# chao1224/GeoSSL

Measured on AMD Instinct MI355X. Metric: molecules/s/GPU SchNet+DDM fwd+bwd (QM9-sized, bs=1024); % HBM roofline, higher is better.
Workload: dtype f32

## Files before the change

### geossl_amd/csrc/ncsn_bwd.hip

```cpp
#include "common.h"
#include "geossl_hip.h"
#include "split.h"
#include "tn.h"

using namespace geossl;

namespace {

constexpr int TR = 32;

#ifdef NB_TIMING
__device__ long long nb_dbg[2 * 32 * 8];
#define NB_MARK(slot)                                                                              \
  do {                                                                                             \
    if (blockIdx.x == 5 && lane == 0 && (wave == 0 || wave == NW) && t - t_begin < 32)             \
      nb_dbg[((wave == 0 ? 0 : 1) * 32 + (t - t_begin)) * 8 + (slot)] = clock64();                 \
  } while (0)
#else
#define NB_MARK(slot) do {} while (0)
#endif

template <int NW>
struct NbLds {
  static constexpr int F = 32 * NW, H = F / 2, KHS = (H + 15) / 16, HMB = (H + 31) / 32, KS = F / 16;
  u32x4* zb;
  u32x4* dz2T;
  u32x4* fT;
  u32x4* dz1r;
  u32x4* abT;
  int4* scal;
  float* pdv;
  float* dep;
  float* wls;
  int* eg;
  int* ef;
  int* ea;
  int* ec;
  __device__ explicit NbLds(uint8_t* smem) {
    zb = reinterpret_cast<u32x4*>(smem);
    dz2T = zb + 2 * KHS * 2 * 64;
    fT = dz2T + HMB * 2 * 2 * 64;
    dz1r = fT + 2 * NW * 2 * 2 * 64;
    abT = dz1r + KS * 2 * 64;
    scal = reinterpret_cast<int4*>(abT + NW * 2 * 2 * 64);
    pdv = reinterpret_cast<float*>(scal + 3 * TR);
    dep = pdv + 3 * TR;
    wls = dep + NW * TR;
    eg = reinterpret_cast<int*>(wls + F);
    ef = eg + 4;
    ea = ef + 2 * NW;
    ec = ea + NW;
  }
  static size_t bytes() {
    return (size_t)(2 * KHS * 2 + HMB * 4 + 2 * NW * 4 + KS * 2 + NW * 4) * 1024 + 3 * TR * sizeof(int4) +
           (size_t)(3 * TR + NW * TR + F) * sizeof(float) + (size_t)(4 + 4 * NW) * sizeof(int);
  }
};

struct NcsnFusedArgs {
  const float* h;
  const int64_t* sei0;
  const int64_t* sei1;
  int S;
  GeosslNcsnWeights w;
  GeosslNcsnSaved sv;
  const int64_t* divisor;
  float out_scale;
  const float* gout;
  float* dfeat;
  float* demb;
  float* grow;
  float* pw1;
  float* pd1;
  float* pb1;
  float* pw2;
  float* pb2;
  float* psm;
};

__device__ __forceinline__ float ldg_off(const float* base, uint32_t byte_off) {
  return *reinterpret_cast<const float*>(reinterpret_cast<const char*>(base) + byte_off);
}
__device__ __forceinline__ int crow4(int r, int k4) { return (r & 3) + 8 * (r >> 2) + k4; }
__device__ __forceinline__ int opaque(int v) {
  asm volatile("" : "+v"(v));
  return v;
}
__device__ __forceinline__ u32x4 pack8(const f32x16& t, int s) {
  u32x4 w;
#pragma unroll
  for (int q = 0; q < 4; ++q) {
    const f16x2 p = {(_Float16)t[8 * s + 2 * q], (_Float16)t[8 * s + 2 * q + 1]};
    w[q] = __builtin_bit_cast(uint32_t, p);
  }
  return w;
}
__device__ __forceinline__ const u32x4& piece(const Frag2& f, int pc) { return pc == 0 ? f.h : f.l; }
__device__ __forceinline__ int scale_exponent(float m) { return max(mag_exponent(m), -40); }
__device__ __forceinline__ float pow2(int e) { return __builtin_amdgcn_ldexpf(1.0f, e); }
constexpr int E_NONE = -100000;

template <int NW, bool ROLE_A>
__device__ __forceinline__ void ncsn_bwd_body(const NcsnFusedArgs& a, const int S, const float* __restrict__ a_h) {
  using L_t = NbLds<NW>;
  constexpr int F = L_t::F, H = L_t::H, KHS = L_t::KHS, HMB = L_t::HMB, KS = L_t::KS, NT = 128 * NW;
  extern __shared__ __attribute__((aligned(16))) uint8_t smem_raw[];
  const L_t L(smem_raw);
  const int tid = threadIdx.x, lane = tid & 63, j = lane & 31, kh = lane >> 5;
  const int wave = __builtin_amdgcn_readfirstlane(tid >> 6);
  const int nb = ROLE_A ? wave : wave - NW;
  const int ntiles = (S + TR - 1) / TR;
  const int per = (ntiles + (int)gridDim.x - 1) / (int)gridDim.x;
  const int t_begin = (int)blockIdx.x * per, t_end = min(ntiles, t_begin + per);
  const float scale = a.out_scale * (a.gout != nullptr ? a.gout[0] : 1.0f) / (float)a.divisor[0];
  const uint32_t col = 32 * nb + j;

  Frag2 wreg[ROLE_A ? KHS : KS];
  f32x16 accw1[ROLE_A ? NW : 1];
  f32x16 accw2[ROLE_A ? 1 : HMB];
  int E1[ROLE_A ? NW : 1];
  int E2 = E_NONE;
  int ew = 0;
  float bsum = 0.0f, dsum = 0.0f;
  u32x4 ident[2];
  float w3r[8];
  float s_w2 = 0.0f, s_w1 = 0.0f, s_b1 = 0.0f, s_g = 0.0f, s_d = 0.0f;
  float iw1 = 0.0f, ib1 = 0.0f, iw2 = 0.0f;
  int e3;
  {
    float m3 = 0.0f;
    for (int i = lane; i < H; i += 64) m3 = fmaxf(m3, fabsf(a.w.o3_w[i]));
    e3 = scale_exponent(wave_max(m3));
  }
  if constexpr (ROLE_A) {
    iw1 = a.w.in_w1[col];
    ib1 = a.w.in_b1[col];
    iw2 = a.w.in_w2[col];
    float raw[KHS][8];
    float wm = 0.0f, csum = 0.0f;
#pragma unroll
    for (int ks = 0; ks < KHS; ++ks)
#pragma unroll
      for (int e = 0; e < 8; ++e) {
        const int m = 16 * ks + 8 * kh + e;
        const float v = m < H ? a.w.o2_w[(size_t)m * F + col] : 0.0f;
        raw[ks][e] = v;
        wm = fmaxf(wm, fabsf(v));
        csum = fmaf(fabsf(v), m < H ? fabsf(a.w.o3_w[m]) : 0.0f, csum);
      }
    ew = scale_exponent(wave_max(wm));
    const float sw = pow2(14 - ew);
#pragma unroll
    for (int ks = 0; ks < KHS; ++ks) wreg[ks] = split8h_scaled(raw[ks], sw);
    csum += __shfl_xor(csum, 32, 64);
    const int ecw = max(mag_exponent(wave_max(csum)), -80);
    if (lane == 0) L.ec[nb] = ecw;
#pragma unroll
    for (int kb = 0; kb < NW; ++kb) {
      E1[kb] = E_NONE;
#pragma unroll
      for (int r = 0; r < 16; ++r) accw1[kb][r] = 0.0f;
    }
#pragma unroll
    for (int s = 0; s < 2; ++s)
#pragma unroll
      for (int q = 0; q < 4; ++q) {
        const int k0 = 16 * s + kperm(2 * q, kh), k1 = 16 * s + kperm(2 * q + 1, kh);
        ident[s][q] = (k0 == j ? 0x3C00u : 0u) | (k1 == j ? 0x3C000000u : 0u);
      }
// ... 18 lines not shown
    }
#pragma unroll
    for (int mb = 0; mb < HMB; ++mb)
#pragma unroll
      for (int r = 0; r < 16; ++r) accw2[mb][r] = 0.0f;
#pragma unroll
    for (int q2 = 0; q2 < 2; ++q2)
#pragma unroll
      for (int q = 0; q < 4; ++q) {
        const int k0 = 16 * q2 + 8 * kh + 2 * q;
        ident[q2][q] = (k0 == j ? 0x3C00u : 0u) | (k0 + 1 == j ? 0x3C000000u : 0u);
      }
  }
  for (int i = tid; i < F; i += NT) L.wls[i] = a.w.o1_w[(size_t)i * (F + 1) + F];

  int sc_u = 0, sc_v = 0;
  float sc_g = 0.0f, sc_e = 0.0f, sc_p = 0.0f;
  int EG = -60;
  auto load_scal = [&](int tt) {
    if constexpr (ROLE_A) {
      if (wave == 0) {
        const int row = min(TR * tt + j, S - 1);
        sc_u = (int)a.sei0[row];
        sc_v = (int)a.sei1[row];
        sc_g = a.sv.gscale[row];
        sc_e = a.sv.emb[row];
        sc_p = a.sv.pd[row];
      }
    }
  };
  auto put_scal = [&](int tt) {
    if constexpr (ROLE_A) {
      if (wave == 0) {
        const int row = TR * tt + lane;
        const bool valid = lane < TR && row < S && tt < t_end;
        const float gr = valid ? pin(sc_g) * scale : 0.0f;
        EG = max(EG, mag_exponent(wave_max(fabsf(gr))));
        if (lane < TR) {
          L.scal[(tt % 3) * TR + lane] = make_int4(sc_u, sc_v, __float_as_int(gr), __float_as_int(sc_e));
          L.pdv[(tt % 3) * TR + lane] = sc_p;
          if (valid) a.grow[row] = gr;
        }
        if (lane == 0) L.eg[tt % 3] = EG;
      }
    }
  };
  float a1raw[16];
  auto request_a1 = [&](int tt, int k4) {
    if constexpr (ROLE_A) {
#pragma unroll
      for (int r = 0; r < 16; ++r)
        a1raw[r] = ldg_off(a.sv.a1, ((uint32_t)min(TR * tt + crow4(r, k4), S - 1) * (uint32_t)F + col) * 4u);
    }
  };
  f32x4 a2raw[2];
  float o3acc[8] = {0.0f, 0.0f, 0.0f, 0.0f, 0.0f, 0.0f, 0.0f, 0.0f};
  auto request_a2 = [&](int tt) {
    if constexpr (!ROLE_A) {
      if (nb < KHS) {
        const uint32_t off = ((uint32_t)min(TR * tt + j, S - 1) * (uint32_t)H + (16 * nb + 8 * kh)) * 4u;
        a2raw[0] = *reinterpret_cast<const f32x4*>(reinterpret_cast<const char*>(a.sv.a2) + off);
        a2raw[1] = *reinterpret_cast<const f32x4*>(reinterpret_cast<const char*>(a.sv.a2) + 16 + off);
      }
    }
  };
  float hu[16], hv[16];
  auto request_gather = [&](int tt, int k4) {
    if constexpr (!ROLE_A) {
      const int2* sc = reinterpret_cast<const int2*>(L.scal + (tt % 3) * TR);
#pragma unroll
      for (int r = 0; r < 16; ++r) {
        const int2 uv = sc[2 * crow4(r, k4)];
        hu[r] = ldg_off(a_h, ((uint32_t)uv.x * (uint32_t)F + col) * 4u);
        hv[r] = ldg_off(a_h, ((uint32_t)uv.y * (uint32_t)F + col) * 4u);
      }
    }
  };
  auto build_zb = [&](int tt) {
    if constexpr (!ROLE_A) {
      if (nb < KHS) {
        const float gr = __int_as_float(L.scal[(tt % 3) * TR + j].z);
        const float sz = pow2(14 - e3 - __builtin_amdgcn_readfirstlane(L.eg[tt % 3]));
        const float av[8] = {a2raw[0].x, a2raw[0].y, a2raw[0].z, a2raw[0].w, a2raw[1].x, a2raw[1].y, a2raw[1].z, a2raw[1].w};
        float v[8];
#pragma unroll
        for (int e = 0; e < 8; ++e) {
          const float a2v = pin(av[e]);
          v[e] = a2v > 0.0f ? gr * w3r[e] : 0.0f;
          o3acc[e] = fmaf(gr, a2v, o3acc[e]);
        }
        const Frag2 f = split8h_scaled(v, sz);
        u32x4* dst = L.zb + (size_t)(((tt & 1) * KHS + nb) * 2) * 64 + lane;
        dst[0] = f.h;
        dst[64] = f.l;
      }
    }
  };
  int EF = -40;
  auto build_fT = [&](int tt) {
    if constexpr (!ROLE_A) {
      float v[16];
      float m = 0.0f;
#pragma unroll
      for (int r = 0; r < 16; ++r) {
        v[r] = pin(hu[r]) + pin(hv[r]);
        m = fmaxf(m, fabsf(v[r]));
      }
      EF = max(EF, mag_exponent(wave_max(m)));
      const float sf = pow2(14 - EF);
      if (lane == 0) L.ef[(tt & 1) * NW + nb] = EF;
#pragma unroll
      for (int s = 0; s < 2; ++s) {
        float vv[8];
#pragma unroll
        for (int e = 0; e < 8; ++e) vv[e] = v[8 * s + e];
        const Frag2 f = split8h_scaled(vv, sf);
        u32x4* dst = L.fT + (size_t)((((tt & 1) * NW + nb) * 2 + s) * 2) * 64 + lane;
        dst[0] = f.h;
        dst[64] = f.l;
      }
    }
  };

  load_scal(t_begin);
  put_scal(t_begin);
  load_scal(t_begin + 1);
  put_scal(t_begin + 1);
  load_scal(t_begin + 2);
  if (t_begin < t_end) {
    request_a1(t_begin, 4 * kh);
    request_a2(t_begin);
  }
  __syncthreads();
  int eC = -80;
#pragma unroll
  for (int i = 0; i < NW; ++i) eC = max(eC, __builtin_amdgcn_readfirstlane(L.ec[i]));
  if (t_begin < t_end) {
    request_gather(t_begin, 4 * kh);
    build_zb(t_begin);
    build_fT(t_begin);
    request_a2(t_begin + 1);
    request_gather(t_begin + 1, 4 * kh);
  }
  int EA = -40;
  const float kA = pow2(e3 + ew - eC - 14);
  for (int t = t_begin; t < t_end; ++t) {
    const int buf = t & 1;
    int k4 = opaque(4 * kh);
    NB_MARK(0);
    lds_barrier();
    NB_MARK(1);
    const int EGt = __builtin_amdgcn_readfirstlane(L.eg[t % 3]);
    if constexpr (ROLE_A) {
      put_scal(t + 2);
      const float kT = pow2(EGt + eC - 14);
      f32x16 acc0, acc1;
#pragma unroll
      for (int r = 0; r < 16; ++r) acc0[r] = acc1[r] = 0.0f;
      {
        const u32x4* zs = L.zb + (size_t)(buf * KHS * 2) * 64 + lane;
        Frag2 a0, an;
        a0.h = zs[0]; a0.l = zs[64];
#pragma unroll
        for (int ks = 0; ks < KHS; ++ks) {
          if (ks + 1 < KHS) {
            const u32x4* s0 = zs + (size_t)((ks + 1) * 2) * 64;
            an.h = s0[0]; an.l = s0[64];
          }
          __builtin_amdgcn_sched_barrier(0);
          mma3x2(acc0, acc1, a0, wreg[ks]);
          __builtin_amdgcn_sched_barrier(0);
          if (ks + 1 < KHS) a0 = an;
        }
      }
      NB_MARK(5);
      float v[16];
      {
        const int4* sc = L.scal + (t % 3) * TR;
        float tb = 0.0f, td = 0.0f, am = 0.0f;
#pragma unroll
        for (int r = 0; r < 16; ++r) {
          a1raw[r] = pin(a1raw[r]);
          v[r] = a1raw[r] > 0.0f ? (acc0[r] + acc1[r]) * kA : 0.0f;
          tb += v[r];
          td = fmaf(v[r], __int_as_float(sc[crow4(r, k4)].w), td);
          am = fmaxf(am, fabsf(a1raw[r]));
        }
        bsum = fmaf(tb, kT, bsum);
        dsum = fmaf(td, kT, dsum);
        EA = max(EA, mag_exponent(wave_max(am)));
      }
      {
        const float sa = pow2(14 - EA);
        if (lane == 0) L.ea[nb] = EA;
#pragma unroll
        for (int s = 0; s < 2; ++s) {
          float vv[8];
#pragma unroll
          for (int e = 0; e < 8; ++e) vv[e] = a1raw[8 * s + e];
          const Frag2 f = split8h_scaled(vv, sa);
          u32x4* dst = L.abT + (size_t)((nb * 2 + s) * 2) * 64 + lane;
          dst[0] = f.h;
          dst[64] = f.l;
        }
      }
      Frag2 da[2];
#pragma unroll
      for (int s = 0; s < 2; ++s) {
        float vv[8];
#pragma unroll
        for (int e = 0; e < 8; ++e) vv[e] = v[8 * s + e];
        da[s] = split8h(vv);
      }
      {
        float wl[16];
#pragma unroll
        for (int r = 0; r < 16; ++r) wl[r] = L.wls[32 * nb + crow4(r, k4)];
        float de = 0.0f;
#pragma unroll
        for (int pc = 1; pc >= 0; --pc) {
          f32x16 tp;
#pragma unroll
          for (int r = 0; r < 16; ++r) tp[r] = 0.0f;
          tp = mfma_f16(piece(da[0], pc), ident[0], tp);
          tp = mfma_f16(piece(da[1], pc), ident[1], tp);
#pragma unroll
          for (int r = 0; r < 16; ++r) de = fmaf(tp[r], wl[r], de);
#pragma unroll
          for (int half = 0; half < 2; ++half)
            L.dz1r[(size_t)((2 * nb + half) * 2 + pc) * 64 + lane] = pack8(tp, half);
        }
        de += __shfl_xor(de, 32, 64);
        if (kh == 0) L.dep[j * NW + nb] = de * kT;
      }
      NB_MARK(6);
#pragma unroll
      for (int kb = 0; kb < NW; ++kb) {
        const int En = EGt + __builtin_amdgcn_readfirstlane(L.ef[buf * NW + kb]);
        if (En != E1[kb]) {
          const float f = pow2(max(E1[kb] - En, -200));
#pragma unroll
          for (int r = 0; r < 16; ++r) accw1[kb][r] *= f;
          E1[kb] = En;
        }
#pragma unroll
        for (int s = 0; s < 2; ++s) {
          const u32x4* s0 = L.fT + (size_t)(((buf * NW + kb) * 2 + s) * 2) * 64 + lane;
          Frag2 bf;
          bf.h = s0[0]; bf.l = s0[64];
          mma3(accw1[kb], da[s], bf);
        }
      }
    } else {
      if (nb < HMB) {
        float tb = 0.0f;
#pragma unroll
        for (int pc = 1; pc >= 0; --pc) {
          f32x16 tp;
#pragma unroll
          for (int r = 0; r < 16; ++r) tp[r] = 0.0f;
#pragma unroll
          for (int q = 0; q < 2; ++q) {
            if (2 * nb + q < KHS) {
              const u32x4* s0 = L.zb + (size_t)((buf * KHS + 2 * nb + q) * 2 + pc) * 64 + lane;
              tp = mfma_f16(s0[0], ident[q], tp);
            }
          }
#pragma unroll
          for (int r = 0; r < 16; ++r) tb += tp[r];
#pragma unroll
          for (int s = 0; s < 2; ++s) L.dz2T[(size_t)((nb * 2 + s) * 2 + pc) * 64 + lane] = pack8(tp, s);
        }
        bsum = fmaf(tb, pow2(EGt + e3 - 14), bsum);
      }
      NB_MARK(5);
      build_zb(t + 1);
      NB_MARK(6);
      build_fT(t + 1);
    }
    k4 = opaque(4 * kh);
    NB_MARK(2);
    lds_barrier();
    NB_MARK(3);
    if constexpr (ROLE_A) {
      request_a1(t + 1, k4);
      load_scal(t + 3);
      {
        const int4* sc = L.scal + (t % 3) * TR;
        const float* pdr = L.pdv + (t % 3) * TR;
#pragma unroll
        for (int i = 0; i < 16; ++i) {
          const int rl = 4 * k4 + i;
          float de = 0.0f;
#pragma unroll
          for (int n2 = 0; n2 < NW; ++n2) de += L.dep[rl * NW + n2];
          const float pd = pdr[rl];
          const float pre = fmaf(iw1, pd, ib1);
          s_w2 = fmaf(de, fmaxf(pre, 0.0f), s_w2);
          const float dp = pre > 0.0f ? de * iw2 : 0.0f;
          s_w1 = fmaf(dp, pd, s_w1);
          s_b1 += dp;
          if (wave == 0 && j == i) {
            s_g += __int_as_float(sc[rl].z);
            s_d += de;
          }
        }
      }
    } else {
      request_a2(t + 2);
      request_gather(t + 2, k4);
      NB_MARK(7);
      f32x16 acc0, acc1;
#pragma unroll
      for (int r = 0; r < 16; ++r) acc0[r] = acc1[r] = 0.0f;
      {
        const u32x4* zs = L.dz1r + lane;
        Frag2 b0, bn;
        b0.h = zs[0]; b0.l = zs[64];
#pragma unroll
        for (int ks = 0; ks < KS; ++ks) {
          if (ks + 1 < KS) {
            const u32x4* s0 = zs + (size_t)((ks + 1) * 2) * 64;
            bn.h = s0[0]; bn.l = s0[64];
          }
          __builtin_amdgcn_sched_barrier(0);
          mma3x2(acc0, acc1, wreg[ks], b0);
          __builtin_amdgcn_sched_barrier(0);
          if (ks + 1 < KS) b0 = bn;
        }
      }
      const float kD = pow2(EGt + eC + ew - 28);
      f32x16 outp;
#pragma unroll
      for (int r = 0; r < 16; ++r) outp[r] = (acc0[r] + acc1[r]) * kD;
      const int row = TR * t + j;
      if (row < S) {
        const uint32_t off = ((uint32_t)row * (uint32_t)F + 32 * nb + 4 * kh) * 4u;
#pragma unroll
        for (int q = 0; q < 4; ++q)
          *reinterpret_cast<f32x4*>(reinterpret_cast<char*>(a.dfeat) + 32 * q + off) =
              f32x4{outp[4 * q], outp[4 * q + 1], outp[4 * q + 2], outp[4 * q + 3]};
        if (nb == 0 && kh == 0) {
          float de = 0.0f;
#pragma unroll
          for (int n2 = 0; n2 < NW; ++n2) de += L.dep[j * NW + n2];
          a.demb[row] = de;
        }
      }
      {
        const int En = EGt + __builtin_amdgcn_readfirstlane(L.ea[nb]);
        if (En != E2) {
          const float f = pow2(max(E2 - En, -200));
#pragma unroll
          for (int mb = 0; mb < HMB; ++mb)
#pragma unroll
            for (int r = 0; r < 16; ++r) accw2[mb][r] *= f;
          E2 = En;
        }
      }
#pragma unroll
      for (int s = 0; s < 2; ++s) {
        const u32x4* sb = L.abT + (size_t)((nb * 2 + s) * 2) * 64 + lane;
        Frag2 bf;
        bf.h = sb[0]; bf.l = sb[64];
#pragma unroll
        for (int mb = 0; mb < HMB; ++mb) {
          const u32x4* s0 = L.dz2T + (size_t)((mb * 2 + s) * 2) * 64 + lane;
          Frag2 af;
          af.h = s0[0]; af.l = s0[64];
          mma3(accw2[mb], af, bf);
        }
      }
    }
    NB_MARK(4);
  }
  const size_t pb = blockIdx.x;
  if constexpr (ROLE_A) {
    float* P1 = a.pw1 + pb * F * F;
#pragma unroll
    for (int kb = 0; kb < NW; ++kb) {
      const float f = pow2(max(E1[kb] + eC - 28, -200));
#pragma unroll
      for (int r = 0; r < 16; ++r) P1[(size_t)(32 * nb + c_row(r, lane)) * F + 32 * kb + j] = accw1[kb][r] * f;
    }
    const float sb = bsum + __shfl_xor(bsum, 32, 64), sd = dsum + __shfl_xor(dsum, 32, 64);
    if (kh == 0) {
      a.pb1[pb * F + col] = sb;
      a.pd1[pb * F + col] = sd;
    }
    float* Ps = a.psm + pb * (H + 3 * F + 2);
    const float t_w2 = s_w2 + __shfl_xor(s_w2, 32, 64);
    const float t_w1 = s_w1 + __shfl_xor(s_w1, 32, 64), t_b1 = s_b1 + __shfl_xor(s_b1, 32, 64);
    if (kh == 0) {
      Ps[H + col] = t_w2;
      Ps[H + F + col] = t_w1;
      Ps[H + 2 * F + col] = t_b1;
    }
    if (wave == 0) {
      const float tg = wave_sum(s_g), td = wave_sum(s_d);
      if (lane == 0) {
        Ps[H + 3 * F] = tg;
        Ps[H + 3 * F + 1] = td;
      }
    }
  } else {
    float* P2 = a.pw2 + pb * H * F;
    const float f = pow2(max(E2 + e3 - 28, -200));
#pragma unroll
    for (int mb = 0; mb < HMB; ++mb)
#pragma unroll
      for (int r = 0; r < 16; ++r) {
        const int m = 32 * mb + c_row(r, lane);
        if (m < H) P2[(size_t)m * F + col] = accw2[mb][r] * f;
      }
    const float sb = bsum + __shfl_xor(bsum, 32, 64);
    if (nb < HMB && kh == 0 && (int)col < H) a.pb2[pb * H + col] = sb;
    if (nb < KHS) {
      float* Ps = a.psm + pb * (H + 3 * F + 2);
#pragma unroll
      for (int e = 0; e < 8; ++e) {
        float v = o3acc[e];
#pragma unroll
        for (int o = 16; o > 0; o >>= 1) v += __shfl_xor(v, o, 64);
        const int m = 16 * nb + 8 * kh + e;
        if (j == 0 && m < H) Ps[m] = v;
      }
    }
  }
}

template <int NW>
__global__ __launch_bounds__(128 * NW) void k_ncsn_bwd_fused(NcsnFusedArgs a) {
  if ((int)(threadIdx.x >> 6) < NW) ncsn_bwd_body<NW, true>(a, a.S, a.h);
  else ncsn_bwd_body<NW, false>(a, a.S, a.h);
}
struct NcsnFusedPair { NcsnFusedArgs a[2]; };
template <int NW>
__global__ __launch_bounds__(128 * NW) void k_ncsn_bwd_fused2(NcsnFusedPair pr, const int32_t* __restrict__ dyn_S,
                                                              const int32_t* __restrict__ dyn_view) {
  const NcsnFusedArgs& a = pr.a[blockIdx.y];
  const int S = dyn_count(a.S, dyn_S);
  const float* h = a.h;
  if (dyn_view != nullptr && blockIdx.y == 1) h += (size_t)(*dyn_view) * (32 * NW);
  if ((int)(threadIdx.x >> 6) < NW) ncsn_bwd_body<NW, true>(a, S, h);
  else ncsn_bwd_body<NW, false>(a, S, h);
}

__device__ __forceinline__ void ncsn_reduce_all_block(const ReduceMulti& m, int nblk, int accumulate,
                                                      const float* __restrict__ psm, int F, const GeosslNcsnGrads& g,
                                                      float (*red)[64]) {
  const int mb = m.xoff[m.nseg];
  if ((int)blockIdx.x < mb) {
    reduce_multi_block(m, nblk, accumulate, red, 0);
    return;
  }
  const int H = F / 2, len = H + 3 * F + 2;
  const int i = ((int)blockIdx.x - mb) * 4 + (int)(threadIdx.x >> 6), lane = threadIdx.x & 63;
  if (i >= len) return;
  float s = 0.0f;
  for (int b = lane; b < nblk; b += 64) s += psm[(size_t)b * len + i];
  s = wave_sum(s);
  if (lane == 0) {
    float* dst;
    if (i < H) dst = g.o3_w + i;
    else if (i < H + F) dst = g.in_w2 + (i - H);
    else if (i < H + 2 * F) dst = g.in_w1 + (i - H - F);
    else if (i < H + 3 * F) dst = g.in_b1 + (i - H - 2 * F);
    else if (i == H + 3 * F) dst = g.o3_b;
    else dst = g.in_b2;
    *dst = accumulate ? *dst + s : s;
  }
}
__global__ __launch_bounds__(256) void k_ncsn_reduce_all(ReduceMulti m, int nblk, int accumulate,
                                                         const float* __restrict__ psm, int F, GeosslNcsnGrads g) {
  __shared__ float red[4][64];
  ncsn_reduce_all_block(m, nblk, accumulate, psm, F, g, red);
}
__global__ __launch_bounds__(256) void k_ncsn_reduce_all2(ReduceMulti m0, ReduceMulti m1, int nblk, int accumulate,
                                                          const float* __restrict__ psm0,
                                                          const float* __restrict__ psm1, int F, GeosslNcsnGrads g0,
                                                          GeosslNcsnGrads g1) {
  __shared__ float red[4][64];
  if (blockIdx.y == 0) ncsn_reduce_all_block(m0, nblk, accumulate, psm0, F, g0, red);
  else ncsn_reduce_all_block(m1, nblk, accumulate, psm1, F, g1, red);
}

inline int fused_blocks(int64_t S) {
  const int64_t ntiles = (S + TR - 1) / TR;
  return (int)(ntiles < 256 ? ntiles : 256);
}

}

#ifdef NB_TIMING
extern "C" int geossl_ncsn_bwd_debug_read(long long* host) {
  return (int)hipMemcpyFromSymbol(host, HIP_SYMBOL(nb_dbg), sizeof(long long) * 2 * 32 * 8);
}
#endif

extern "C" int64_t geossl_ddm_loss_bwd_fused_workspace_floats(int64_t S, int F) {
  const int64_t nb = fused_blocks(S), H = F / 2;
  return nb * ((int64_t)F * F + 2 * F + H * F + H + (H + 3 * F + 2));
}

extern "C" int geossl_ddm_loss_bwd_fused(const float* h, const int64_t* sei0, const int64_t* sei1, int64_t S, int64_t N,
                                         int F, const GeosslNcsnWeights* w, const GeosslNcsnSaved* saved,
                                         const int64_t* stats_divisor, float out_scale, const float* gout, float* dfeat,
                                         float* demb, float* grow, const GeosslNcsnGrads* grads, float* workspace,
                                         int accumulate, hipStream_t stream) {
  if (S <= 0) return 0;
  if (F != 32 && F != 64 && F != 128) return (int)hipErrorInvalidValue;
  if (S * (int64_t)F * 4 >= ((int64_t)1 << 32) || N * (int64_t)F * 4 >= ((int64_t)1 << 32)) return (int)hipErrorInvalidValue;
  const int nb = fused_blocks(S), H = F / 2;
  NcsnFusedArgs a;
  a.h = h; a.sei0 = sei0; a.sei1 = sei1; a.S = (int)S; a.w = *w; a.sv = *saved; a.divisor = stats_divisor;
  a.out_scale = out_scale; a.gout = gout; a.dfeat = dfeat; a.demb = demb; a.grow = grow;
  a.pw1 = workspace;
  a.pd1 = a.pw1 + (size_t)nb * F * F;
  a.pb1 = a.pd1 + (size_t)nb * F;
  a.pw2 = a.pb1 + (size_t)nb * F;
  a.pb2 = a.pw2 + (size_t)nb * H * F;
  a.psm = a.pb2 + (size_t)nb * H;
#define LAUNCH(NWV)                                                                                      \
  do {                                                                                                   \
    allow_big_lds(&k_ncsn_bwd_fused<NWV>);                                                               \
// ... 91 lines not shown
```

### geossl_amd/csrc/ncsn_rows.hip

```cpp
#include "common.h"
#include "geossl_hip.h"
#include "split.h"

using namespace geossl;

namespace {

struct RowIn {
  int64_t u, v;
  float sigma, d, eps;
};

template <int NMB>
__device__ __forceinline__ void ncsn_fwd_body(const float* __restrict__ h, const int64_t* __restrict__ batch,
                                              const int64_t* __restrict__ sei0, const int64_t* __restrict__ sei1,
                                              int S, const float* __restrict__ distance,
                                              const int64_t* __restrict__ noise_level,
                                              const float* __restrict__ dist_noise, const GeosslNcsnWeights& w,
                                              float anneal_power, float* __restrict__ loss_e,
                                              const GeosslNcsnSaved& sv, float* __restrict__ loss_part) {
  constexpr int F = 32 * NMB, H = F / 2, HMB = (H + 31) / 32, HP = 32 * HMB, KS = F / 16;
  extern __shared__ __attribute__((aligned(16))) uint8_t smem_raw[];
  u32x4* W1f = reinterpret_cast<u32x4*>(smem_raw);
  u32x4* W2f = W1f + NMB * KS * 3 * 64;
  float* b1s = reinterpret_cast<float*>(W2f + HMB * KS * 3 * 64);
  float* wls = b1s + F;
  float* b2s = wls + F;
  float* w3s = b2s + HP;
  float* iw1 = w3s + HP;
  float* ib1 = iw1 + F;
  float* iw2 = ib1 + F;
  float* lred = iw2 + F;
  const int tid = threadIdx.x, lane = tid & 63, wave = tid >> 6, j = lane & 31, kh = lane >> 5;
  const int nrb = (S + 31) / 32;
  float lsum = 0.0f;
  auto load_row = [&](int rb) {
    RowIn r;
    const int rowc = min(32 * rb + j, S - 1);
    r.u = sei0[rowc];
    r.v = sei1[rowc];
    r.sigma = w.sigmas[noise_level[batch[r.u]]];
    r.d = distance[rowc];
    r.eps = dist_noise[rowc];
    return r;
  };
  int rb = blockIdx.x + gridDim.x * wave;
  RowIn cur;
  if (rb < nrb) cur = load_row(rb);
#ifdef NCSN_STAGE_UNROLL
#pragma unroll
#endif
  for (int i = tid; i < NMB * KS * 64; i += 512) {
    const int ln = i & 63, ks = (i >> 6) % KS, mb = i / (64 * KS);
    const float* row = w.o1_w + (size_t)(32 * mb + (ln & 31)) * (F + 1) + 16 * ks + 8 * (ln >> 5);
    float v[8];
#pragma unroll
    for (int e = 0; e < 8; ++e) v[e] = row[e];
    const Frag3 f = split8(v);
    u32x4* dst = W1f + ((size_t)(mb * KS + ks) * 3) * 64 + ln;
    dst[0] = f.h;
    dst[64] = f.m;
    dst[128] = f.l;
  }
#ifdef NCSN_STAGE_UNROLL
#pragma unroll
#endif
  for (int i = tid; i < HMB * KS * 64; i += 512) {
    const int ln = i & 63, ks = (i >> 6) % KS, mb = i / (64 * KS);
    const int m = 32 * mb + (ln & 31);
    const float* row = w.o2_w + (size_t)min(m, H - 1) * F + 16 * ks + 4 * (ln >> 5);
    const f32x4 lo = *reinterpret_cast<const f32x4*>(row), hi = *reinterpret_cast<const f32x4*>(row + 8);
    float v[8] = {lo.x, lo.y, lo.z, lo.w, hi.x, hi.y, hi.z, hi.w};
    if (m >= H) {
#pragma unroll
      for (int e = 0; e < 8; ++e) v[e] = 0.0f;
    }
    const Frag3 f = split8(v);
    u32x4* dst = W2f + ((size_t)(mb * KS + ks) * 3) * 64 + ln;
    dst[0] = f.h;
    dst[64] = f.m;
    dst[128] = f.l;
  }
  for (int i = tid; i < F; i += 512) {
    b1s[i] = w.o1_b[i];
    wls[i] = w.o1_w[(size_t)i * (F + 1) + F];
    iw1[i] = w.in_w1[i];
    ib1[i] = w.in_b1[i];
    iw2[i] = w.in_w2[i];
  }
  for (int i = tid; i < HP; i += 512) {
    b2s[i] = i < H ? w.o2_b[i] : 0.0f;
    w3s[i] = i < H ? w.o3_w[i] : 0.0f;
  }
  __syncthreads();
  const float ib2 = w.in_b2[0], b3 = w.o3_b[0];
  for (; rb < nrb; rb += gridDim.x * 8) {
    const int row = 32 * rb + j;
    const bool valid = row < S;
    const RowIn in = cur;
    f32x4 gq[2][4];
    auto gather = [&](int ks, f32x4 (&g)[4]) {
      const float* hu = h + (size_t)in.u * F + 16 * ks + 8 * kh;
      const float* hv = h + (size_t)in.v * F + 16 * ks + 8 * kh;
      g[0] = *reinterpret_cast<const f32x4*>(hu);
      g[1] = *reinterpret_cast<const f32x4*>(hu + 4);
      g[2] = *reinterpret_cast<const f32x4*>(hv);
      g[3] = *reinterpret_cast<const f32x4*>(hv + 4);
    };
    gather(0, gq[0]);
    if (rb + gridDim.x * 8 < nrb) cur = load_row(rb + gridDim.x * 8);
    const float pd = add_rn(in.d, mul_rn(in.eps, in.sigma));
    float e = 0.0f;
#pragma unroll 4
    for (int k = kh * (F / 2); k < (kh + 1) * (F / 2); k += 4) {
      const f32x4 a = *reinterpret_cast<const f32x4*>(iw1 + k), b = *reinterpret_cast<const f32x4*>(ib1 + k);
      const f32x4 c = *reinterpret_cast<const f32x4*>(iw2 + k);
      e = fmaf(c.x, fmaxf(fmaf(a.x, pd, b.x), 0.0f), e);
      e = fmaf(c.y, fmaxf(fmaf(a.y, pd, b.y), 0.0f), e);
      e = fmaf(c.z, fmaxf(fmaf(a.z, pd, b.z), 0.0f), e);
      e = fmaf(c.w, fmaxf(fmaf(a.w, pd, b.w), 0.0f), e);
    }
    e += __shfl_xor(e, 32, 64);
    const float emb = e + ib2;
    f32x16 acc1[NMB];
#pragma unroll
    for (int mb = 0; mb < NMB; ++mb)
#pragma unroll
      for (int q = 0; q < 4; ++q) {
        const f32x4 b = *reinterpret_cast<const f32x4*>(b1s + 32 * mb + 8 * q + 4 * kh);
        const f32x4 wl = *reinterpret_cast<const f32x4*>(wls + 32 * mb + 8 * q + 4 * kh);
        acc1[mb][4 * q] = fmaf(emb, wl.x, b.x);
        acc1[mb][4 * q + 1] = fmaf(emb, wl.y, b.y);
        acc1[mb][4 * q + 2] = fmaf(emb, wl.z, b.z);
        acc1[mb][4 * q + 3] = fmaf(emb, wl.w, b.w);
      }
#pragma unroll
    for (int ks = 0; ks < KS; ++ks) {
      if (ks + 1 < KS) gather(ks + 1, gq[(ks + 1) & 1]);
      const f32x4(&g)[4] = gq[ks & 1];
      const float v[8] = {g[0].x + g[2].x, g[0].y + g[2].y, g[0].z + g[2].z, g[0].w + g[2].w,
                          g[1].x + g[3].x, g[1].y + g[3].y, g[1].z + g[3].z, g[1].w + g[3].w};
      const Frag3 bf = split8(v);
      Frag3 af[NMB];
#pragma unroll
      for (int mb = 0; mb < NMB; ++mb) {
        const u32x4* src = W1f + ((size_t)(mb * KS + ks) * 3) * 64 + lane;
        af[mb].h = src[0];
        af[mb].m = src[64];
        af[mb].l = src[128];
      }
#pragma unroll
      for (int mb = 0; mb < NMB; ++mb) acc1[mb] = mfma_bf16(af[mb].l, bf.h, acc1[mb]);
#pragma unroll
      for (int mb = 0; mb < NMB; ++mb) acc1[mb] = mfma_bf16(af[mb].h, bf.l, acc1[mb]);
#pragma unroll
      for (int mb = 0; mb < NMB; ++mb) acc1[mb] = mfma_bf16(af[mb].m, bf.m, acc1[mb]);
#pragma unroll
      for (int mb = 0; mb < NMB; ++mb) acc1[mb] = mfma_bf16(af[mb].m, bf.h, acc1[mb]);
#pragma unroll
      for (int mb = 0; mb < NMB; ++mb) acc1[mb] = mfma_bf16(af[mb].h, bf.m, acc1[mb]);
#pragma unroll
      for (int mb = 0; mb < NMB; ++mb) acc1[mb] = mfma_bf16(af[mb].h, bf.h, acc1[mb]);
      __builtin_amdgcn_sched_barrier(0);
    }
    Frag3 tb[KS];
    {
      float* arow = sv.a1 != nullptr ? sv.a1 + (size_t)row * F + 4 * kh : nullptr;
#pragma unroll
      for (int mb = 0; mb < NMB; ++mb)
#pragma unroll
        for (int half = 0; half < 2; ++half) {
          float v[8];
#pragma unroll
          for (int e2 = 0; e2 < 8; ++e2) v[e2] = fmaxf(acc1[mb][8 * half + e2], 0.0f);
          if (arow != nullptr && valid) {
            *reinterpret_cast<f32x4*>(arow + 32 * mb + 16 * half) = f32x4{v[0], v[1], v[2], v[3]};
            *reinterpret_cast<f32x4*>(arow + 32 * mb + 16 * half + 8) = f32x4{v[4], v[5], v[6], v[7]};
          }
          tb[2 * mb + half] = split8(v);
          __builtin_amdgcn_sched_barrier(0);
        }
    }
    float sc = 0.0f;
#pragma unroll
    for (int mb = 0; mb < HMB; ++mb) {
      f32x16 acc2;
#pragma unroll
      for (int q = 0; q < 4; ++q) {
        const f32x4 b = *reinterpret_cast<const f32x4*>(b2s + 32 * mb + 8 * q + 4 * kh);
        acc2[4 * q] = b.x;
        acc2[4 * q + 1] = b.y;
        acc2[4 * q + 2] = b.z;
        acc2[4 * q + 3] = b.w;
      }
      Frag3 af, an;
      {
        const u32x4* src = W2f + ((size_t)(mb * KS) * 3) * 64 + lane;
        af.h = src[0]; af.m = src[64]; af.l = src[128];
      }
#pragma unroll
      for (int ks = 0; ks < KS; ++ks) {
        if (ks + 1 < KS) {
          const u32x4* src = W2f + ((size_t)(mb * KS + ks + 1) * 3) * 64 + lane;
          an.h = src[0]; an.m = src[64]; an.l = src[128];
        }
        __builtin_amdgcn_sched_barrier(0);
        mma6(acc2, af, tb[ks]);
        __builtin_amdgcn_sched_barrier(0);
        if (ks + 1 < KS) af = an;
      }
      float* a2row = sv.a2 != nullptr ? sv.a2 + (size_t)row * H + 32 * mb + 4 * kh : nullptr;
#pragma unroll
      for (int q = 0; q < 4; ++q) {
        const f32x4 w3 = *reinterpret_cast<const f32x4*>(w3s + 32 * mb + 8 * q + 4 * kh);
        const f32x4 a = f32x4{fmaxf(acc2[4 * q], 0.0f), fmaxf(acc2[4 * q + 1], 0.0f), fmaxf(acc2[4 * q + 2], 0.0f),
                              fmaxf(acc2[4 * q + 3], 0.0f)};
        sc = fmaf(a.x, w3.x, sc);
        sc = fmaf(a.y, w3.y, sc);
        sc = fmaf(a.z, w3.z, sc);
        sc = fmaf(a.w, w3.w, sc);
        if (a2row != nullptr && valid && 32 * mb + 8 * q + 4 * kh < H) *reinterpret_cast<f32x4*>(a2row + 8 * q) = a;
      }
    }
    sc += __shfl_xor(sc, 32, 64);
    const float out = sc + b3;
    const float inv_sigma = 1.0f / in.sigma;
    const float score = out * inv_sigma;
    const float target = (-1.0f / (in.sigma * in.sigma)) * (pd - in.d);
    const float diff = score - target;
    const float pw = powf(in.sigma, anneal_power);
    if (valid && kh == 0) {
      const float le = (0.5f * (diff * diff)) * pw;
      loss_e[row] = le;
      lsum += le;
      if (sv.pd != nullptr) {
        sv.pd[row] = pd;
        sv.emb[row] = emb;
        sv.gscale[row] = diff * pw * inv_sigma;
      }
    }
  }
  if (loss_part != nullptr) {
    lsum = wave_sum(lsum);
    if (lane == 0) lred[wave] = lsum;
    __syncthreads();
    if (tid == 0) {
      float t = 0.0f;
      for (int i = 0; i < 8; ++i) t += lred[i];
      loss_part[blockIdx.x] = t;
    }
    if (blockIdx.x == 0)
      for (int i = (int)gridDim.x + tid; i < GEOSSL_LOSS_PARTIALS; i += 512) loss_part[i] = 0.0f;
  }
}

template <int NMB>
__global__ __launch_bounds__(512) void k_ncsn_fwd(const float* __restrict__ h, const int64_t* __restrict__ batch,
                                                  const int64_t* __restrict__ sei0, const int64_t* __restrict__ sei1,
                                                  int S, const float* __restrict__ distance,
                                                  const int64_t* __restrict__ noise_level,
                                                  const float* __restrict__ dist_noise, GeosslNcsnWeights w,
                                                  float anneal_power, float* __restrict__ loss_e,
                                                  GeosslNcsnSaved sv, float* __restrict__ loss_part) {
  ncsn_fwd_body<NMB>(h, batch, sei0, sei1, S, distance, noise_level, dist_noise, w, anneal_power, loss_e, sv, loss_part);
}
struct NcsnFwdHead {
  const float* h;
  const float* distance;
  const int64_t* noise_level;
  const float* dist_noise;
  GeosslNcsnWeights w;
  GeosslNcsnSaved sv;
  float anneal_power;
  float* loss_e;
  float* loss_part;
};
struct NcsnFwdPair { NcsnFwdHead a[2]; };
template <int NMB>
__global__ __launch_bounds__(512) void k_ncsn_fwd2(NcsnFwdPair pr, const int64_t* __restrict__ batch,
                                                   const int64_t* __restrict__ sei0, const int64_t* __restrict__ sei1,
                                                   int S, const int32_t* __restrict__ dyn_S,
                                                   const int32_t* __restrict__ dyn_view) {
  const NcsnFwdHead& a = pr.a[blockIdx.y];
  const float* h = a.h;
  if (dyn_view != nullptr && blockIdx.y == 1) h += (size_t)(*dyn_view) * (32 * NMB);
  ncsn_fwd_body<NMB>(h, batch, sei0, sei1, dyn_count(S, dyn_S), a.distance, a.noise_level, a.dist_noise, a.w,
                     a.anneal_power, a.loss_e, a.sv, a.loss_part);
}

template <int NMB>
__global__ __launch_bounds__(512) void k_ncsn_bwd_rows(GeosslNcsnWeights w, GeosslNcsnSaved sv, int S,
                                                       const int64_t* __restrict__ divisor, float out_scale,
                                                       const float* __restrict__ gout, float* __restrict__ dz1,
                                                       float* __restrict__ dfeat, float* __restrict__ demb,
                                                       float* __restrict__ grow) {
  constexpr int F = 32 * NMB, H = F / 2, HP = 32 * ((H + 31) / 32), KS = F / 16, KH = H / 16;
  extern __shared__ __attribute__((aligned(16))) uint8_t smem_raw[];
  u32x4* W2t = reinterpret_cast<u32x4*>(smem_raw);
  u32x4* W1t = W2t + NMB * KH * 3 * 64;
  float* wls = reinterpret_cast<float*>(W1t + NMB * KS * 3 * 64);
  float* w3s = wls + F;
  const int tid = threadIdx.x, lane = tid & 63, wave = tid >> 6, j = lane & 31, kh = lane >> 5;
  for (int i = tid; i < NMB * KH * 64; i += 512) {
    const int ln = i & 63, ks = (i >> 6) % KH, mb = i / (64 * KH);
    const float* col = w.o2_w + (size_t)(16 * ks + 8 * (ln >> 5)) * F + 32 * mb + (ln & 31);
    float v[8];
#pragma unroll
    for (int e = 0; e < 8; ++e) v[e] = col[(size_t)e * F];
    const Frag3 f = split8(v);
    u32x4* dst = W2t + ((size_t)(mb * KH + ks) * 3) * 64 + ln;
    dst[0] = f.h;
    dst[64] = f.m;
    dst[128] = f.l;
  }
  for (int i = tid; i < NMB * KS * 64; i += 512) {
    const int ln = i & 63, ks = (i >> 6) % KS, mb = i / (64 * KS);
    const float* col = w.o1_w + 32 * mb + (ln & 31);
    float v[8];
#pragma unroll
    for (int e = 0; e < 8; ++e) v[e] = col[(size_t)(16 * ks + kperm(e, ln >> 5)) * (F + 1)];
    const Frag3 f = split8(v);
    u32x4* dst = W1t + ((size_t)(mb * KS + ks) * 3) * 64 + ln;
    dst[0] = f.h;
    dst[64] = f.m;
    dst[128] = f.l;
  }
  for (int i = tid; i < F; i += 512) wls[i] = w.o1_w[(size_t)i * (F + 1) + F];
  for (int i = tid; i < HP; i += 512) w3s[i] = i < H ? w.o3_w[i] : 0.0f;
  __syncthreads();
  const float scale = out_scale * (gout != nullptr ? gout[0] : 1.0f) / (float)divisor[0];
  const int nrb = (S + 31) / 32;
  for (int rb = blockIdx.x + gridDim.x * wave; rb < nrb; rb += gridDim.x * 8) {
    const int row = 32 * rb + j;
    const bool valid = row < S;
    const size_t rowc = (size_t)min(row, S - 1);
    const float gr = valid ? sv.gscale[rowc] * scale : 0.0f;
    if (valid && kh == 0) grow[row] = gr;
    Frag3 zb[KH];
    {
      const float* a2row = sv.a2 + rowc * H + 8 * kh;
      f32x4 a2v[KH][2];
#pragma unroll
      for (int ks = 0; ks < KH; ++ks) {
        a2v[ks][0] = *reinterpret_cast<const f32x4*>(a2row + 16 * ks);
        a2v[ks][1] = *reinterpret_cast<const f32x4*>(a2row + 16 * ks + 4);
      }
#pragma unroll
      for (int ks = 0; ks < KH; ++ks) {
        const f32x4 w0 = *reinterpret_cast<const f32x4*>(w3s + 16 * ks + 8 * kh);
        const f32x4 w1 = *reinterpret_cast<const f32x4*>(w3s + 16 * ks + 8 * kh + 4);
        const f32x4 a0 = a2v[ks][0], a1 = a2v[ks][1];
        const float v[8] = {a0.x > 0.0f ? gr * w0.x : 0.0f, a0.y > 0.0f ? gr * w0.y : 0.0f,
                            a0.z > 0.0f ? gr * w0.z : 0.0f, a0.w > 0.0f ? gr * w0.w : 0.0f,
                            a1.x > 0.0f ? gr * w1.x : 0.0f, a1.y > 0.0f ? gr * w1.y : 0.0f,
                            a1.z > 0.0f ? gr * w1.z : 0.0f, a1.w > 0.0f ? gr * w1.w : 0.0f};
        zb[ks] = split8(v);
      }
// ... 212 lines not shown
```

Before: 414,400.

## Software-pipeline LDS fragment loads and staged row-index gathers across iterations

The backward kernel now loads LDS fragments (fT, zb, dz2T, abT) and exponent scalars into registers before the MFMA chains, double-buffering the fT loads. It also hoists the per-row s_g/s_d accumulation out of the 16-iteration loop. The rows kernel splits the dependent index chain (edge index, batch, noise level, sigma) into stages that are interleaved with the K loop. It prefetches the next row's first two h gathers with triple buffering, so global latency overlaps with MFMA work. In exchange, register pressure rises, which may lower occupancy or cause spills.

```diff
diff --git a/geossl_amd/csrc/ncsn_bwd.hip b/geossl_amd/csrc/ncsn_bwd.hip
--- a/geossl_amd/csrc/ncsn_bwd.hip
+++ b/geossl_amd/csrc/ncsn_bwd.hip
@@ -11,10 +11,10 @@
 
 #ifdef NB_TIMING
 __device__ long long nb_dbg[2 * 32 * 8];
-#define NB_MARK(slot)                                                                              \
-  do {                                                                                             \
-    if (blockIdx.x == 5 && lane == 0 && (wave == 0 || wave == NW) && t - t_begin < 32)             \
-      nb_dbg[((wave == 0 ? 0 : 1) * 32 + (t - t_begin)) * 8 + (slot)] = clock64();                 \
+#define NB_MARK(slot)                                                                                      \
+  do {                                                                                                     \
+    if (blockIdx.x == 5 && blockIdx.y == 0 && lane == 0 && (wave == 0 || wave == NW) && t - t_begin < 32)  \
+      nb_dbg[((wave == 0 ? 0 : 1) * 32 + (t - t_begin)) * 8 + (slot)] = clock64();                         \
   } while (0)
 #else
 #define NB_MARK(slot) do {} while (0)
@@ -339,6 +339,21 @@
     NB_MARK(1);
     const int EGt = __builtin_amdgcn_readfirstlane(L.eg[t % 3]);
     if constexpr (ROLE_A) {
+      int EFt[NW];
+      {
+        const int* efp = L.ef + buf * NW;
+        if constexpr (NW == 4) {
+          const int4 e = *reinterpret_cast<const int4*>(efp);
+          EFt[0] = e.x; EFt[1] = e.y; EFt[2] = e.z; EFt[3] = e.w;
+        } else if constexpr (NW == 2) {
+          const int2 e = *reinterpret_cast<const int2*>(efp);
+          EFt[0] = e.x; EFt[1] = e.y;
+        } else {
+          EFt[0] = efp[0];
+        }
+#pragma unroll
+        for (int kb = 0; kb < NW; ++kb) EFt[kb] = __builtin_amdgcn_readfirstlane(EFt[kb]);
+      }
       put_scal(t + 2);
       const float kT = pow2(EGt + eC - 14);
       f32x16 acc0, acc1;
@@ -421,9 +436,20 @@
         if (kh == 0) L.dep[j * NW + nb] = de * kT;
       }
       NB_MARK(6);
+      Frag2 fb[2][2];
+      auto load_fT = [&](int kb, Frag2 (&f)[2]) {
+#pragma unroll
+        for (int s = 0; s < 2; ++s) {
+          const u32x4* s0 = L.fT + (size_t)(((buf * NW + kb) * 2 + s) * 2) * 64 + lane;
+          f[s].h = s0[0]; f[s].l = s0[64];
+        }
+      };
+      load_fT(0, fb[0]);
 #pragma unroll
       for (int kb = 0; kb < NW; ++kb) {
-        const int En = EGt + __builtin_amdgcn_readfirstlane(L.ef[buf * NW + kb]);
+        if (kb + 1 < NW) load_fT(kb + 1, fb[(kb + 1) & 1]);
+        __builtin_amdgcn_sched_barrier(0);
+        const int En = EGt + EFt[kb];
         if (En != E1[kb]) {
           const float f = pow2(max(E1[kb] - En, -200));
 #pragma unroll
@@ -431,16 +457,18 @@
           E1[kb] = En;
         }
 #pragma unroll
-        for (int s = 0; s < 2; ++s) {
-          const u32x4* s0 = L.fT + (size_t)(((buf * NW + kb) * 2 + s) * 2) * 64 + lane;
-          Frag2 bf;
-          bf.h = s0[0]; bf.l = s0[64];
-          mma3(accw1[kb], da[s], bf);
-        }
+        for (int s = 0; s < 2; ++s) mma3(accw1[kb], da[s], fb[kb & 1][s]);
       }
     } else {
       if (nb < HMB) {
         float tb = 0.0f;
+        u32x4 zf[2][2];
+#pragma unroll
+        for (int pc = 1; pc >= 0; --pc)
+#pragma unroll
+          for (int q = 0; q < 2; ++q)
+            if (KHS == 2 * HMB || 2 * nb + q < KHS)
+              zf[pc][q] = L.zb[(size_t)((buf * KHS + 2 * nb + q) * 2 + pc) * 64 + lane];
 #pragma unroll
         for (int pc = 1; pc >= 0; --pc) {
           f32x16 tp;
@@ -448,10 +476,7 @@
           for (int r = 0; r < 16; ++r) tp[r] = 0.0f;
 #pragma unroll
           for (int q = 0; q < 2; ++q) {
-            if (2 * nb + q < KHS) {
-              const u32x4* s0 = L.zb + (size_t)((buf * KHS + 2 * nb + q) * 2 + pc) * 64 + lane;
-              tp = mfma_f16(s0[0], ident[q], tp);
-            }
+            if (KHS == 2 * HMB || 2 * nb + q < KHS) tp = mfma_f16(zf[pc][q], ident[q], tp);
           }
 #pragma unroll
           for (int r = 0; r < 16; ++r) tb += tp[r];
@@ -475,6 +500,14 @@
       {
         const int4* sc = L.scal + (t % 3) * TR;
         const float* pdr = L.pdv + (t % 3) * TR;
+        if (wave == 0 && j < 16) {
+          const int rl = 4 * k4 + j;
+          float de = 0.0f;
+#pragma unroll
+          for (int n2 = 0; n2 < NW; ++n2) de += L.dep[rl * NW + n2];
+          s_g += __int_as_float(sc[rl].z);
+          s_d += de;
+        }
 #pragma unroll
         for (int i = 0; i < 16; ++i) {
           const int rl = 4 * k4 + i;
@@ -487,10 +520,6 @@
           const float dp = pre > 0.0f ? de * iw2 : 0.0f;
           s_w1 = fmaf(dp, pd, s_w1);
           s_b1 += dp;
-          if (wave == 0 && j == i) {
-            s_g += __int_as_float(sc[rl].z);
-            s_d += de;
-          }
         }
       }
     } else {
@@ -534,8 +563,21 @@
           a.demb[row] = de;
         }
       }
+      const int EAt = L.ea[nb];
+      Frag2 w2b[2], w2a[HMB][2];
+#pragma unroll
+      for (int s = 0; s < 2; ++s) {
+        const u32x4* sb = L.abT + (size_t)((nb * 2 + s) * 2) * 64 + lane;
+        w2b[s].h = sb[0]; w2b[s].l = sb[64];
+#pragma unroll
+        for (int mb = 0; mb < HMB; ++mb) {
+          const u32x4* s0 = L.dz2T + (size_t)((mb * 2 + s) * 2) * 64 + lane;
+          w2a[mb][s].h = s0[0]; w2a[mb][s].l = s0[64];
+        }
+      }
+      __builtin_amdgcn_sched_barrier(0);
       {
-        const int En = EGt + __builtin_amdgcn_readfirstlane(L.ea[nb]);
+        const int En = EGt + __builtin_amdgcn_readfirstlane(EAt);
         if (En != E2) {
           const float f = pow2(max(E2 - En, -200));
 #pragma unroll
@@ -546,18 +588,9 @@
         }
       }
 #pragma unroll
-      for (int s = 0; s < 2; ++s) {
-        const u32x4* sb = L.abT + (size_t)((nb * 2 + s) * 2) * 64 + lane;
-        Frag2 bf;
-        bf.h = sb[0]; bf.l = sb[64];
-#pragma unroll
-        for (int mb = 0; mb < HMB; ++mb) {
-          const u32x4* s0 = L.dz2T + (size_t)((mb * 2 + s) * 2) * 64 + lane;
-          Frag2 af;
-          af.h = s0[0]; af.l = s0[64];
-          mma3(accw2[mb], af, bf);
-        }
-      }
+      for (int s = 0; s < 2; ++s)
+#pragma unroll
+        for (int mb = 0; mb < HMB; ++mb) mma3(accw2[mb], w2a[mb][s], w2b[s]);
     }
     NB_MARK(4);
   }
diff --git a/geossl_amd/csrc/ncsn_rows.hip b/geossl_amd/csrc/ncsn_rows.hip
--- a/geossl_amd/csrc/ncsn_rows.hip
+++ b/geossl_amd/csrc/ncsn_rows.hip
@@ -31,22 +31,40 @@
   float* ib1 = iw1 + F;
   float* iw2 = ib1 + F;
   float* lred = iw2 + F;
-  const int tid = threadIdx.x, lane = tid & 63, wave = tid >> 6, j = lane & 31, kh = lane >> 5;
+  const int tid = threadIdx.x, lane = tid & 63, j = lane & 31, kh = lane >> 5;
+  const int wave = __builtin_amdgcn_readfirstlane(tid >> 6);
   const int nrb = (S + 31) / 32;
   float lsum = 0.0f;
-  auto load_row = [&](int rb) {
-    RowIn r;
-    const int rowc = min(32 * rb + j, S - 1);
-    r.u = sei0[rowc];
-    r.v = sei1[rowc];
-    r.sigma = w.sigmas[noise_level[batch[r.u]]];
-    r.d = distance[rowc];
-    r.eps = dist_noise[rowc];
-    return r;
+  RowIn cur;
+  int64_t cur_b = 0, cur_l = 0;
+  auto row_stage = [&](int stage, int rowc) {
+    if (stage == 0) {
+      cur.u = sei0[rowc];
+      cur.v = sei1[rowc];
+      cur.d = distance[rowc];
+      cur.eps = dist_noise[rowc];
+    } else if (stage == 1) {
+      cur_b = batch[cur.u];
+    } else if (stage == 2) {
+      cur_l = noise_level[cur_b];
+    } else {
+      cur.sigma = w.sigmas[cur_l];
+    }
   };
+  f32x4 gq[3][4];
+  auto gather = [&](const int64_t u, const int64_t v, int ks, f32x4 (&g)[4]) {
+    const float* hu = h + (size_t)u * F + 16 * ks + 8 * kh;
+    const float* hv = h + (size_t)v * F + 16 * ks + 8 * kh;
+    g[0] = *reinterpret_cast<const f32x4*>(hu);
+    g[1] = *reinterpret_cast<const f32x4*>(hu + 4);
+    g[2] = *reinterpret_cast<const f32x4*>(hv);
+    g[3] = *reinterpret_cast<const f32x4*>(hv + 4);
+  };
+  constexpr int GL0 = ((KS - 1) / 3) * 3, GL1 = ((KS - 2) / 3) * 3 + 1;
   int rb = blockIdx.x + gridDim.x * wave;
-  RowIn cur;
-  if (rb < nrb) cur = load_row(rb);
+  const bool any = rb < nrb;
+  const int row0 = min(32 * rb + j, S - 1);
+  if (any) row_stage(0, row0);
 #ifdef NCSN_STAGE_UNROLL
 #pragma unroll
 #endif
@@ -62,6 +80,7 @@
     dst[64] = f.m;
     dst[128] = f.l;
   }
+  if (any) row_stage(1, row0);
 #ifdef NCSN_STAGE_UNROLL
 #pragma unroll
 #endif
@@ -81,6 +100,7 @@
     dst[64] = f.m;
     dst[128] = f.l;
   }
+  if (any) row_stage(2, row0);
   for (int i = tid; i < F; i += 512) {
     b1s[i] = w.o1_b[i];
     wls[i] = w.o1_w[(size_t)i * (F + 1) + F];
@@ -92,23 +112,22 @@
     b2s[i] = i < H ? w.o2_b[i] : 0.0f;
     w3s[i] = i < H ? w.o3_w[i] : 0.0f;
   }
+  if (any) {
+    row_stage(3, row0);
+    gather(cur.u, cur.v, 0, gq[0]);
+    gather(cur.u, cur.v, 1, gq[1]);
+  }
   __syncthreads();
   const float ib2 = w.in_b2[0], b3 = w.o3_b[0];
   for (; rb < nrb; rb += gridDim.x * 8) {
     const int row = 32 * rb + j;
     const bool valid = row < S;
     const RowIn in = cur;
-    f32x4 gq[2][4];
-    auto gather = [&](int ks, f32x4 (&g)[4]) {
-      const float* hu = h + (size_t)in.u * F + 16 * ks + 8 * kh;
-      const float* hv = h + (size_t)in.v * F + 16 * ks + 8 * kh;
-      g[0] = *reinterpret_cast<const f32x4*>(hu);
-      g[1] = *reinterpret_cast<const f32x4*>(hu + 4);
-      g[2] = *reinterpret_cast<const f32x4*>(hv);
-      g[3] = *reinterpret_cast<const f32x4*>(hv + 4);
-    };
-    gather(0, gq[0]);
-    if (rb + gridDim.x * 8 < nrb) cur = load_row(rb + gridDim.x * 8);
+    const int rb_n = rb + (int)gridDim.x * 8;
+    const int row_n = min(32 * (rb_n < nrb ? rb_n : rb) + j, S - 1);
+    row_stage(0, row_n);
+    if (KS > 2) gather(in.u, in.v, 2, gq[2]);
+    __builtin_amdgcn_sched_barrier(0);
     const float pd = add_rn(in.d, mul_rn(in.eps, in.sigma));
     float e = 0.0f;
 #pragma unroll 4
@@ -136,8 +155,14 @@
       }
 #pragma unroll
     for (int ks = 0; ks < KS; ++ks) {
-      if (ks + 1 < KS) gather(ks + 1, gq[(ks + 1) & 1]);
-      const f32x4(&g)[4] = gq[ks & 1];
+      if (ks >= 1 && ks + 2 < KS) gather(in.u, in.v, ks + 2, gq[(ks + 2) % 3]);
+      if (ks == GL0 + 1) gather(cur.u, cur.v, 0, gq[0]);
+      if (ks == GL1 + 1) gather(cur.u, cur.v, 1, gq[1]);
+      if (ks == KS / 4) row_stage(1, row_n);
+      if (ks == KS / 2) row_stage(2, row_n);
+      if (ks == (3 * KS) / 4) row_stage(3, row_n);
+      __builtin_amdgcn_sched_barrier(0);
+      const f32x4(&g)[4] = gq[ks % 3];
       const float v[8] = {g[0].x + g[2].x, g[0].y + g[2].y, g[0].z + g[2].z, g[0].w + g[2].w,
                           g[1].x + g[3].x, g[1].y + g[3].y, g[1].z + g[3].z, g[1].w + g[3].w};
       const Frag3 bf = split8(v);
@@ -163,6 +188,9 @@
       for (int mb = 0; mb < NMB; ++mb) acc1[mb] = mfma_bf16(af[mb].h, bf.h, acc1[mb]);
       __builtin_amdgcn_sched_barrier(0);
     }
+    if (GL0 + 1 == KS) gather(cur.u, cur.v, 0, gq[0]);
+    if (GL1 + 1 == KS) gather(cur.u, cur.v, 1, gq[1]);
+    __builtin_amdgcn_sched_barrier(0);
     Frag3 tb[KS];
     {
       float* arow = sv.a1 != nullptr ? sv.a1 + (size_t)row * F + 4 * kh : nullptr;
```

Measured after the change: 417,500 (median of 6 runs). About the same (+0.7%).

## Software-pipeline NCSN row gathers, next-row metadata loads and W1 fragment LDS reads

Applied to the files above, without the earlier changes.

Replaces the row-level prefetch with a deeper pipeline. Feature gathers now run two k-steps ahead in a triple buffer, and the next row's first two gathers are issued before the second layer. The dependent metadata chain for the next row (edge index, batch, noise level, sigma) is split across k-steps so each latency hides behind MFMA work. W1 fragments are loaded piece by piece, interleaved with the MFMA groups, and LDS addresses are pinned to a few base registers, which lowers register pressure and exposes overlap. The cost is more complex scheduling, extra live registers for three gather buffers, and clamped speculative loads on the last iteration.

```diff
diff --git a/geossl_amd/csrc/ncsn_rows.hip b/geossl_amd/csrc/ncsn_rows.hip
--- a/geossl_amd/csrc/ncsn_rows.hip
+++ b/geossl_amd/csrc/ncsn_rows.hip
@@ -94,21 +94,40 @@
   }
   __syncthreads();
   const float ib2 = w.in_b2[0], b3 = w.o3_b[0];
+  f32x4 gq[3][4];
+  auto gather = [&](const RowIn& r, int ks, f32x4 (&g)[4]) {
+    const float* hu = h + (size_t)r.u * F + 16 * ks + 8 * kh;
+    const float* hv = h + (size_t)r.v * F + 16 * ks + 8 * kh;
+    g[0] = *reinterpret_cast<const f32x4*>(hu);
+    g[1] = *reinterpret_cast<const f32x4*>(hu + 4);
+    g[2] = *reinterpret_cast<const f32x4*>(hv);
+    g[3] = *reinterpret_cast<const f32x4*>(hv + 4);
+  };
+  int wslot[3] = {lane, lane + 4096, lane + 8192};
+#pragma unroll
+  for (int i = 0; i < 3; ++i) asm volatile("" : "+v"(wslot[i]));
+  auto wfrag = [&](int idx) -> u32x4 { return W1f[wslot[idx >> 12] + (idx & 4095)]; };
+  auto w1_piece = [&](int ks, int piece, u32x4 (&p)[NMB]) {
+#pragma unroll
+    for (int mb = 0; mb < NMB; ++mb) p[mb] = wfrag(((mb * KS + ks) * 3 + piece) * 64);
+  };
+  if (rb < nrb) {
+    gather(cur, 0, gq[0]);
+    gather(cur, 1, gq[1]);
+  }
+  constexpr int KB = KS / 4, KN = KS / 2, KG = (3 * KS) / 4;
   for (; rb < nrb; rb += gridDim.x * 8) {
     const int row = 32 * rb + j;
     const bool valid = row < S;
     const RowIn in = cur;
-    f32x4 gq[2][4];
-    auto gather = [&](int ks, f32x4 (&g)[4]) {
-      const float* hu = h + (size_t)in.u * F + 16 * ks + 8 * kh;
-      const float* hv = h + (size_t)in.v * F + 16 * ks + 8 * kh;
-      g[0] = *reinterpret_cast<const f32x4*>(hu);
-      g[1] = *reinterpret_cast<const f32x4*>(hu + 4);
-      g[2] = *reinterpret_cast<const f32x4*>(hv);
-      g[3] = *reinterpret_cast<const f32x4*>(hv + 4);
-    };
-    gather(0, gq[0]);
-    if (rb + gridDim.x * 8 < nrb) cur = load_row(rb + gridDim.x * 8);
+    const bool more = rb + gridDim.x * 8 < nrb;
+    const int rowcn = min(32 * (more ? rb + (int)gridDim.x * 8 : rb) + j, S - 1);
+    RowIn nx;
+    nx.u = sei0[rowcn];
+    nx.v = sei1[rowcn];
+    nx.d = distance[rowcn];
+    nx.eps = dist_noise[rowcn];
+    int64_t nb = 0, nl = 0;
     const float pd = add_rn(in.d, mul_rn(in.eps, in.sigma));
     float e = 0.0f;
 #pragma unroll 4
@@ -134,34 +153,51 @@
         acc1[mb][4 * q + 2] = fmaf(emb, wl.z, b.z);
         acc1[mb][4 * q + 3] = fmaf(emb, wl.w, b.w);
       }
+    u32x4 pa[NMB], pb[NMB];
+    w1_piece(0, 2, pa);
 #pragma unroll
     for (int ks = 0; ks < KS; ++ks) {
-      if (ks + 1 < KS) gather(ks + 1, gq[(ks + 1) & 1]);
-      const f32x4(&g)[4] = gq[ks & 1];
+      if (ks + 2 < KS) gather(in, ks + 2, gq[(ks + 2) % 3]);
+      if (ks == KB) {
+        uint32_t ulo = (uint32_t)nx.u, uhi = (uint32_t)((uint64_t)nx.u >> 32);
+        asm volatile("" : "+v"(ulo), "+v"(uhi));
+        nx.u = (int64_t)(((uint64_t)uhi << 32) | ulo);
+        nb = batch[nx.u];
+      }
+      if (ks == KN) nl = noise_level[nb];
+      if (ks == KG) nx.sigma = w.sigmas[nl];
+      const f32x4(&g)[4] = gq[ks % 3];
       const float v[8] = {g[0].x + g[2].x, g[0].y + g[2].y, g[0].z + g[2].z, g[0].w + g[2].w,
                           g[1].x + g[3].x, g[1].y + g[3].y, g[1].z + g[3].z, g[1].w + g[3].w};
       const Frag3 bf = split8(v);
-      Frag3 af[NMB];
-#pragma unroll
-      for (int mb = 0; mb < NMB; ++mb) {
-        const u32x4* src = W1f + ((size_t)(mb * KS + ks) * 3) * 64 + lane;
-        af[mb].h = src[0];
-        af[mb].m = src[64];
-        af[mb].l = src[128];
-      }
-#pragma unroll
-      for (int mb = 0; mb < NMB; ++mb) acc1[mb] = mfma_bf16(af[mb].l, bf.h, acc1[mb]);
-#pragma unroll
-      for (int mb = 0; mb < NMB; ++mb) acc1[mb] = mfma_bf16(af[mb].h, bf.l, acc1[mb]);
-#pragma unroll
-      for (int mb = 0; mb < NMB; ++mb) acc1[mb] = mfma_bf16(af[mb].m, bf.m, acc1[mb]);
-#pragma unroll
-      for (int mb = 0; mb < NMB; ++mb) acc1[mb] = mfma_bf16(af[mb].m, bf.h, acc1[mb]);
-#pragma unroll
-      for (int mb = 0; mb < NMB; ++mb) acc1[mb] = mfma_bf16(af[mb].h, bf.m, acc1[mb]);
-#pragma unroll
-      for (int mb = 0; mb < NMB; ++mb) acc1[mb] = mfma_bf16(af[mb].h, bf.h, acc1[mb]);
-      __builtin_amdgcn_sched_barrier(0);
+      __builtin_amdgcn_sched_barrier(0);
+      w1_piece(ks, 0, pb);
+#pragma unroll
+      for (int mb = 0; mb < NMB; ++mb) acc1[mb] = mfma_bf16(pa[mb], bf.h, acc1[mb]);
+      __builtin_amdgcn_sched_barrier(0);
+      w1_piece(ks, 1, pa);
+#pragma unroll
+      for (int mb = 0; mb < NMB; ++mb) acc1[mb] = mfma_bf16(pb[mb], bf.l, acc1[mb]);
+      __builtin_amdgcn_sched_barrier(0);
+#pragma unroll
+      for (int mb = 0; mb < NMB; ++mb) acc1[mb] = mfma_bf16(pa[mb], bf.m, acc1[mb]);
+      __builtin_amdgcn_sched_barrier(0);
+#pragma unroll
+      for (int mb = 0; mb < NMB; ++mb) acc1[mb] = mfma_bf16(pa[mb], bf.h, acc1[mb]);
+      __builtin_amdgcn_sched_barrier(0);
+      if (ks + 1 < KS) w1_piece(ks + 1, 2, pa);
+#pragma unroll
+      for (int mb = 0; mb < NMB; ++mb) acc1[mb] = mfma_bf16(pb[mb], bf.m, acc1[mb]);
+      __builtin_amdgcn_sched_barrier(0);
+#pragma unroll
+      for (int mb = 0; mb < NMB; ++mb) acc1[mb] = mfma_bf16(pb[mb], bf.h, acc1[mb]);
+      __builtin_amdgcn_sched_barrier(0);
+    }
+    asm volatile("" : "+v"(nx.sigma));
+    cur = nx;
+    if (more) {
+      gather(cur, 0, gq[0]);
+      gather(cur, 1, gq[1]);
     }
     Frag3 tb[KS];
     {
@@ -194,15 +230,16 @@
         acc2[4 * q + 3] = b.w;
       }
       Frag3 af, an;
+      constexpr int W2I = NMB * KS * 3 * 64;
       {
-        const u32x4* src = W2f + ((size_t)(mb * KS) * 3) * 64 + lane;
-        af.h = src[0]; af.m = src[64]; af.l = src[128];
+        const int i0 = W2I + (mb * KS) * 3 * 64;
+        af.h = wfrag(i0); af.m = wfrag(i0 + 64); af.l = wfrag(i0 + 128);
       }
 #pragma unroll
       for (int ks = 0; ks < KS; ++ks) {
         if (ks + 1 < KS) {
-          const u32x4* src = W2f + ((size_t)(mb * KS + ks + 1) * 3) * 64 + lane;
-          an.h = src[0]; an.m = src[64]; an.l = src[128];
+          const int i1 = W2I + (mb * KS + ks + 1) * 3 * 64;
+          an.h = wfrag(i1); an.m = wfrag(i1 + 64); an.l = wfrag(i1 + 128);
         }
         __builtin_amdgcn_sched_barrier(0);
         mma6(acc2, af, tb[ks]);
```

Result: no change. 413,400 before, 415,100 after, median of 6 (+0.4%).
